# NikNazarov/TorchPIV

Hardware: AMD Instinct MI355X
Metric: image-pairs/sec at 4 MP, wind=64 ov=32 2-pass CWS; % HBM roofline (higher is better)
Workload: dtype u32 exact sums + f64 / f32

## Files before the change

### torchpiv_amd/csrc/xcorr_tile.hpp

```cpp
#pragma once
#include <hip/hip_runtime.h>
#include <stdint.h>

#include "fft_inreg.hpp"
#include "piv_kernels.h"

namespace tpiv {

template <int WS, bool PLANAR_ = false>
struct TileGeo {
    static constexpr int WPW = 64 / WS;
    static constexpr int TS = WS > 32 ? 32 : WS;
    static constexpr int PITCH = TS + 1;
    static constexpr int NT = 64 / TS;
    static constexpr int TILE = TS * PITCH;
    static constexpr bool PLANAR = PLANAR_;
    static constexpr int HROWS = WS / 2 + 1;
    static constexpr int HTILE = HROWS * PITCH;
    static constexpr int LDS_FLOATS = NT * TILE * (PLANAR ? 1 : 2);
    static constexpr int MAP_PITCH = WS + 1;
    static constexpr int NDW = WS / 4;
};

template <int CTRL>
__device__ __forceinline__ int dpp_i(int v) {
    return __builtin_amdgcn_update_dpp(0, v, CTRL, 0xF, 0xF, true);
}
template <int CTRL>
__device__ __forceinline__ float dpp_f(float v) {
    return __int_as_float(dpp_i<CTRL>(__float_as_int(v)));
}
constexpr int DPP_XOR1 = 0xB1;
constexpr int DPP_XOR2 = 0x4E;
constexpr int DPP_HALF_MIRROR = 0x141;
constexpr int DPP_ROW_MIRROR = 0x140;

template <int HALF>
__device__ __forceinline__ void partner2(int a, int& pa) {
    if constexpr (HALF == 1) pa = dpp_i<DPP_XOR1>(a);
    else if constexpr (HALF == 2) pa = dpp_i<DPP_XOR2>(a);
    else if constexpr (HALF == 4) pa = dpp_i<DPP_HALF_MIRROR>(a);
    else if constexpr (HALF == 8) pa = dpp_i<DPP_ROW_MIRROR>(a);
}

template <int WS, typename T, typename OP>
__device__ __forceinline__ T grp_reduce(T v, OP op) {
    static_assert(sizeof(T) == 4 || sizeof(T) == 8, "one or two dwords");
    constexpr int NW = sizeof(T) / 4;
    union U {
        T t;
        int w[NW];
    };
    static_for<0, 4>([&](auto sc) TPIV_LAMBDA_INLINE {
        constexpr int half = 1 << decltype(sc)::value;
        if constexpr (half < WS) {
            U a, b;
            a.t = v;
#pragma unroll
            for (int q = 0; q < NW; ++q) partner2<half>(a.w[q], b.w[q]);
            v = op(v, b.t);
        }
    });
    if constexpr (WS >= 32) {
        U a, x, y;
        a.t = v;
#pragma unroll
        for (int q = 0; q < NW; ++q) {
            auto r = __builtin_amdgcn_permlane16_swap((unsigned)a.w[q], (unsigned)a.w[q], false, false);
            x.w[q] = (int)r[0];
            y.w[q] = (int)r[1];
        }
        v = op(x.t, y.t);
    }
    if constexpr (WS >= 64) {
        U a, x, y;
        a.t = v;
#pragma unroll
        for (int q = 0; q < NW; ++q) {
            auto r = __builtin_amdgcn_permlane32_swap((unsigned)a.w[q], (unsigned)a.w[q], false, false);
            x.w[q] = (int)r[0];
            y.w[q] = (int)r[1];
        }
        v = op(x.t, y.t);
    }
    return v;
}

template <int WS>
__device__ __forceinline__ float grp_sum(float v) {
    return grp_reduce<WS>(v, [](float a, float b) TPIV_LAMBDA_INLINE { return a + b; });
}

template <int WS>
__device__ __forceinline__ float grp_min(float v) {
    return grp_reduce<WS>(v, [](float a, float b) TPIV_LAMBDA_INLINE { return fminf(a, b); });
}

__device__ __forceinline__ float fetch_clamped_t(const uint8_t* __restrict__ f, long long q, int HW) {
    q = q < 0 ? 0 : (q > (long long)(HW - 1) ? (long long)(HW - 1) : q);
    return (float)f[q];
}

__device__ __forceinline__ int f2i_sat_t(float v) {
    v = fminf(fmaxf(v, -1073741824.f), 1073741824.f);
    return (int)v;
}

template <int K, int N>
__device__ __forceinline__ float byte_f(const uint32_t (&d)[N]) {
    return (float)((d[K >> 2] >> (8 * (K & 3))) & 0xffu);
}

template <int N>
__device__ __forceinline__ void load_dwords(const uint8_t* __restrict__ p, uint32_t (&d)[N]) {
    __builtin_memcpy(&d[0], p, 4 * N);
}

__device__ __forceinline__ float bilerp_ref(float f11, float f21, float f12, float f22, float wx_up,
                                            float wx_dn, float wy_up, float wy_dn, bool degenerate) {
#pragma clang fp contract(off)
    float r = (f11 * wx_up) * wy_up;
    r = r + (f21 * wx_dn) * wy_up;
    r = r + (f12 * wx_up) * wy_dn;
    r = r + (f22 * wx_dn) * wy_dn;
    return degenerate ? f11 : r;
}

__device__ __forceinline__ float bilerp_ref_m(float f11, float f21, float f12, float f22, float wx_up,
                                              float wx_dn, float wy_up, float wy_dn, unsigned degenerate_mask) {
#pragma clang fp contract(off)
    float r = (f11 * wx_up) * wy_up;
    r = r + (f21 * wx_dn) * wy_up;
    r = r + (f12 * wx_up) * wy_dn;
    r = r + (f22 * wx_dn) * wy_dn;
    const unsigned bits = (degenerate_mask & __float_as_uint(f11)) | (~degenerate_mask & __float_as_uint(r));
    return __uint_as_float(bits);
}

#ifdef TPIV_STAMPS
#define TPIV_STAMP_DECL unsigned long long st_acc[16] = {}; unsigned long long st_prev = 0; unsigned st_iter = 0; \
    unsigned long long st_t0 = __builtin_amdgcn_s_memtime(), st_r0 = __builtin_amdgcn_s_memrealtime();
#define TPIV_STAMP_START                                                                  \
    do {                                                                                  \
        __builtin_amdgcn_sched_barrier(0);                                                \
        asm volatile("s_memtime %0\n\ts_waitcnt lgkmcnt(0)" : "=s"(st_prev)::"memory");    \
        __builtin_amdgcn_sched_barrier(0);                                                \
    } while (0)
#define TPIV_STAMP(i)                                                                     \
    do {                                                                                  \
        unsigned long long st_t;                                                          \
        __builtin_amdgcn_sched_barrier(0);                                                \
        asm volatile("s_memtime %0\n\ts_waitcnt lgkmcnt(0)" : "=s"(st_t)::"memory");       \
        __builtin_amdgcn_sched_barrier(0);                                                \
        st_acc[i] += st_t - st_prev;                                                      \
        st_prev = st_t;                                                                   \
    } while (0)
#define TPIV_STAMP_FLUSH(pp)                                                              \
    do {                                                                                  \
        if ((pp).stamps != nullptr && threadIdx.x == 0) {                                 \
            for (int q_ = 0; q_ < 16; ++q_) atomicAdd(&(pp).stamps[q_], st_acc[q_]);      \
            atomicAdd(&(pp).stamps[16], (unsigned long long)st_iter);                     \
            atomicAdd(&(pp).stamps[17], __builtin_amdgcn_s_memtime() - st_t0);            \
            atomicAdd(&(pp).stamps[18], __builtin_amdgcn_s_memrealtime() - st_r0);        \
        }                                                                                 \
    } while (0)
#else
#define TPIV_STAMP_DECL
#define TPIV_STAMP_START
#define TPIV_STAMP(i)
#define TPIV_STAMP_FLUSH(pp)
#endif

__device__ __forceinline__ int fast_div(int n, unsigned magic, int shift) {
    return (int)(((unsigned long long)(unsigned)n * magic) >> shift);
}
inline void fast_div_setup(unsigned d, unsigned& magic, int& shift) {
    int s_ = 0;
    while ((1ull << s_) < d) ++s_;
    shift = 31 + s_;
    magic = (unsigned)(((1ull << shift) + d - 1) / d);
}

__device__ __forceinline__ int fresh_lane() {
    int l = (int)__builtin_amdgcn_mbcnt_hi(~0u, __builtin_amdgcn_mbcnt_lo(~0u, 0u));
    asm volatile("" : "+v"(l));
    return l;
}

__device__ __forceinline__ void wave_sync() {
    __builtin_amdgcn_fence(__ATOMIC_ACQ_REL, "wavefront");
    __builtin_amdgcn_wave_barrier();
}

template <int WS, bool PLANAR, bool NOSWAP = false>
__device__ __forceinline__ void transpose_tile(cf (&a)[WS], float* lds, int lane) {
    using G = TileGeo<WS, PLANAR>;
    constexpr int P = G::PITCH;
    static_assert(!NOSWAP || WS == 64, "the swap-free form is a 64x64 one");
    cf* tile = reinterpret_cast<cf*>(lds);
    if constexpr (PLANAR && WS > 32) {
        if constexpr (!NOSWAP) {
            static_for<0, 32>([&](auto kc) TPIV_LAMBDA_INLINE {
                constexpr int k = decltype(kc)::value;
                constexpr int lo = FFT_POS<k, WS>, hi = FFT_POS<k + 32, WS>;
                auto rx = __builtin_amdgcn_permlane32_swap(__float_as_uint(a[lo].x), __float_as_uint(a[hi].x),
                                                           false, false);
                auto ry = __builtin_amdgcn_permlane32_swap(__float_as_uint(a[lo].y), __float_as_uint(a[hi].y),
                                                           false, false);
                a[lo].x = __uint_as_float(rx[0]);
                a[hi].x = __uint_as_float(rx[1]);
                a[lo].y = __uint_as_float(ry[0]);
                a[hi].y = __uint_as_float(ry[1]);
            });
        }
        float* t = lds + (lane >> 5) * G::TILE;
        const float* t2 = NOSWAP ? lds + ((lane >> 5) ^ 1) * G::TILE : t;
        const int i = lane & 31;
        auto plane = [&](auto comp) TPIV_LAMBDA_INLINE {
            constexpr bool Y = decltype(comp)::value;
            float lowhalf[32];
            wave_sync();
            static_for<0, 32>([&](auto kc) TPIV_LAMBDA_INLINE {
                constexpr int k = decltype(kc)::value;
                constexpr int src = FFT_POS<k, WS>;
                t[i * P + k] = Y ? a[src].y : a[src].x;
            });
            wave_sync();
#pragma unroll
            for (int r = 0; r < 32; ++r) lowhalf[r] = t[r * P + i];
            wave_sync();
            static_for<0, 32>([&](auto kc) TPIV_LAMBDA_INLINE {
                constexpr int k = decltype(kc)::value;
                constexpr int src = FFT_POS<k + 32, WS>;
                t[i * P + k] = Y ? a[src].y : a[src].x;
            });
            wave_sync();
#pragma unroll
            for (int r = 0; r < 32; ++r) {
                if constexpr (Y) {
                    a[32 + r].y = t2[r * P + i];
                    a[r].y = lowhalf[r];
                } else {
                    a[32 + r].x = t2[r * P + i];
                    a[r].x = lowhalf[r];
                }
            }
        };
        plane(std::false_type{});
        plane(std::true_type{});
    } else if constexpr (PLANAR) {
        float* t = lds + (lane / WS) * G::TILE;
        const int i = lane % WS;
        wave_sync();
        static_for<0, WS>([&](auto kc) TPIV_LAMBDA_INLINE {
            constexpr int k = decltype(kc)::value;
            t[i * P + k] = a[FFT_POS<k, WS>].x;
        });
        wave_sync();
#pragma unroll
        for (int r = 0; r < WS; ++r) a[r].x = t[r * P + i];
        wave_sync();
        static_for<0, WS>([&](auto kc) TPIV_LAMBDA_INLINE {
            constexpr int k = decltype(kc)::value;
            t[i * P + k] = a[FFT_POS<k, WS>].y;
        });
        wave_sync();
#pragma unroll
        for (int r = 0; r < WS; ++r) a[r].y = t[r * P + i];
    } else if constexpr (WS <= 32) {
        cf* t = tile + (lane / WS) * G::TILE;
        const int i = lane % WS;
        wave_sync();
        static_for<0, WS>([&](auto kc) TPIV_LAMBDA_INLINE {
            constexpr int k = decltype(kc)::value;
            t[i * P + k] = a[FFT_POS<k, WS>];
        });
        wave_sync();
#pragma unroll
        for (int r = 0; r < WS; ++r) a[r] = t[r * P + i];
    } else {
        static_assert(NOSWAP, "the complex 64x64 tile (the CWS kernel at two wavefronts per SIMD) is swap-free");
        cf* t = tile + (lane >> 5) * G::TILE;
        const int i = lane & 31;
        cf lowhalf[32];
        wave_sync();
        static_for<0, 32>([&](auto kc) TPIV_LAMBDA_INLINE {
            constexpr int k = decltype(kc)::value;
            t[i * P + k] = a[FFT_POS<k, WS>];
        });
        wave_sync();
#pragma unroll
        for (int r = 0; r < 32; ++r) lowhalf[r] = t[r * P + i];
        wave_sync();
        static_for<0, 32>([&](auto kc) TPIV_LAMBDA_INLINE {
            constexpr int k = decltype(kc)::value;
            t[i * P + k] = a[FFT_POS<k + 32, WS>];
        });
        wave_sync();
        const cf* t2 = tile + ((lane >> 5) ^ 1) * G::TILE;
#pragma unroll
        for (int r = 0; r < 32; ++r) a[32 + r] = t2[r * P + i];
#pragma unroll
        for (int r = 0; r < 32; ++r) a[r] = lowhalf[r];
    }
}

template <int WS, bool PLANAR>
__device__ __forceinline__ void transpose_half(const cf (&a)[WS], cf (&g)[WS / 2 + 1], float* lds, int lane) {
    static_assert(WS <= 32 || WS == 64, "one tile per window");
    using G = TileGeo<WS, PLANAR>;
    constexpr int P = G::PITCH, M = WS / 2;
    const int i = lane % WS;
    if constexpr (WS == 64) {
        static_assert(!PLANAR, "planar 64x64 tiles run the paired half inverse");
        constexpr int Q = M + 1;
        static_assert(WS * Q * 2 <= G::LDS_FLOATS, "half-spectrum plane fits the tile");
        cf b[WS];
        static_for<0, WS>([&](auto kc) TPIV_LAMBDA_INLINE {
            constexpr int k = decltype(kc)::value;
            b[k] = a[FFT_POS<k, WS>];
            asm volatile("" : "+v"(b[k].x), "+v"(b[k].y));
        });
        wave_sync();
        cf* t = reinterpret_cast<cf*>(lds);
        if (i <= M) {
            static_for<0, WS>([&](auto kc) TPIV_LAMBDA_INLINE {
                constexpr int k = decltype(kc)::value;
                t[k * Q + i] = b[k];
            });
        }
        wave_sync();
#pragma unroll
        for (int r = 0; r <= M; ++r) g[r] = t[i * Q + r];
    } else if constexpr (PLANAR) {
        float* t = lds + (lane / WS) * G::HTILE;
        wave_sync();
        if (i <= M) {
            static_for<0, WS>([&](auto kc) TPIV_LAMBDA_INLINE {
                constexpr int k = decltype(kc)::value;
                t[i * P + k] = a[FFT_POS<k, WS>].x;
            });
        }
        wave_sync();
#pragma unroll
        for (int r = 0; r <= M; ++r) g[r].x = t[r * P + i];
        wave_sync();
        if (i <= M) {
            static_for<0, WS>([&](auto kc) TPIV_LAMBDA_INLINE {
                constexpr int k = decltype(kc)::value;
                t[i * P + k] = a[FFT_POS<k, WS>].y;
            });
        }
        wave_sync();
#pragma unroll
        for (int r = 0; r <= M; ++r) g[r].y = t[r * P + i];
    } else {
        cf* t = reinterpret_cast<cf*>(lds) + (lane / WS) * G::HTILE;
        wave_sync();
        if (i <= M) {
            static_for<0, WS>([&](auto kc) TPIV_LAMBDA_INLINE {
                constexpr int k = decltype(kc)::value;
                t[i * P + k] = a[FFT_POS<k, WS>];
            });
        }
        wave_sync();
#pragma unroll
        for (int r = 0; r <= M; ++r) g[r] = t[r * P + i];
    }
}

template <int WS, bool PLANAR>
__device__ __forceinline__ void transpose_half_pairs(const cf (&h)[WS / 2], cf (&g)[WS / 2 + 1], float* lds, int lane) {
    static_assert(PLANAR && (WS == 32 || WS == 64), "planar tiles of 32 and 64");
    using G = TileGeo<WS, PLANAR>;
    constexpr int M = WS / 2, Q = M + 1;
    static_assert(64 * Q <= G::LDS_FLOATS, "the half-spectrum plane fits the tile");
    const int r = lane % WS;
    float* t = lds + (lane / WS) * (WS * Q);
    const bool odd = r > M;
    constexpr bool ZERO_ODD = WS == 32;
    const bool up = odd || (r == 0 && ZERO_ODD) || (r == M && !ZERO_ODD);
    float* wp = t + (odd ? WS - r : r) + (up ? Q : 0);
    const float sy = odd ? -1.0f : 1.0f;
    cf b[M];
    static_for<0, M>([&](auto mc) TPIV_LAMBDA_INLINE {
        constexpr int m = decltype(mc)::value;
        b[m] = h[FFT_POS<m, M>];
        asm volatile("" : "+v"(b[m].x), "+v"(b[m].y));
    });
    const int y = lane % WS;
    const float* rd = t + y * Q;
    const float* r0 = t + ((y & ~1) + (ZERO_ODD ? 1 : 0)) * Q;
    const float* rm = t + ((y & ~1) + (ZERO_ODD ? 0 : 1)) * Q + M;
    wave_sync();
    static_for<0, M>([&](auto mc) TPIV_LAMBDA_INLINE {
        constexpr int m = decltype(mc)::value;
        wp[2 * Q * m] = b[m].x;
    });
    wave_sync();
    g[0].x = r0[0];
#pragma unroll
    for (int k = 1; k < M; ++k) g[k].x = rd[k];
    g[M].x = rm[0];
    wave_sync();
    static_for<0, M>([&](auto mc) TPIV_LAMBDA_INLINE {
        constexpr int m = decltype(mc)::value;
        wp[2 * Q * m] = b[m].y * sy;
    });
    wave_sync();
    g[0].y = r0[0];
#pragma unroll
    for (int k = 1; k < M; ++k) g[k].y = rd[k];
    g[M].y = rm[0];
    if (y & 1) {
        g[0].x = g[0].y;
        g[M].x = g[M].y;
    }
}

struct ItemGeom {
    int pair, win, y0, x0;
    int active;
    size_t fidx;
};

template <int WS, int MODE>
struct RawRows;
template <int WS>
struct RawRows<WS, MODE_PASS1> {
    uint32_t a[WS / 4], b[WS / 4];
};
template <int WS>
struct RawRows<WS, MODE_DWS> {
    uint32_t a[WS / 4], b[WS / 4];
    long long qa, qb;
    int reg;
    int cls;
    int fix;
};
template <int WS>
struct CoopGeo {
    static constexpr int NROW = WS + 1;
    static constexpr int RPG = (WS + 1 + 15) / 16;
    static constexpr int LOADED = 16 * RPG;
    static constexpr int T = NROW * RPG;
    static constexpr int NCH = (T + WS - 1) / WS;
    static constexpr int PITCH4 = RPG | 1;
    static constexpr int PATCH4 = NROW * PITCH4;
    static constexpr int BLOCK4 = (2 * PATCH4 + 15) / 16 * 16;
    static constexpr int FLOATS = (64 / WS) * BLOCK4 * 4;
    static constexpr int LDS_FLOATS = FLOATS + (64 / WS) * (WS + 1) * 4;
    static_assert(RPG <= PITCH4, "patch row pitch");
    __device__ static __forceinline__ void chunk(int ci, int& j, int& part) {
        if constexpr (RPG == 2) {
            j = ci >> 1;
            part = ci & 1;
        } else if constexpr (RPG == 3) {
            j = (ci * 171) >> 9;
            part = ci - 3 * j;
        } else {
            static_assert(RPG == 5, "chunks per row");
            j = (ci * 205) >> 10;
            part = ci - 5 * j;
        }
    }
};
template <int WS>
struct CoopOff {
    int o[CoopGeo<WS>::NCH];
    __device__ __forceinline__ void init(int r, int W) {
#pragma unroll
        for (int k = 0; k < CoopGeo<WS>::NCH; ++k) {
            int j, part;
            CoopGeo<WS>::chunk(r + WS * k, j, part);
            o[k] = r + WS * k < CoopGeo<WS>::T ? j * W + 16 * part : 0;
        }
    }
};
template <int WS>
struct RawRows<WS, MODE_CWS> {
    uint32_t ca[CoopGeo<WS>::NCH][4], cb[CoopGeo<WS>::NCH][4];
    int reg;
    int cls;
    int fix;
};

struct CwsRow {
    float wya_up, wya_dn, wyb_up, wyb_dn;
    int dya, uya, dyb, uyb;
    int ydeg_a, ydeg_b;
};
__device__ __forceinline__ CwsRow cws_row(int gy, float vy) {
    CwsRow c;
    const float gyf = (float)gy;
    const float nya = gyf - vy, nyb = gyf + vy;
    const float uya_f = ceilf(nya), dya_f = floorf(nya);
    const float uyb_f = ceilf(nyb), dyb_f = floorf(nyb);
    c.uya = f2i_sat_t(uya_f);
    c.dya = f2i_sat_t(dya_f);
    c.uyb = f2i_sat_t(uyb_f);
    c.dyb = f2i_sat_t(dyb_f);
    c.wya_up = uya_f - nya;
    c.wya_dn = nya - dya_f;
// ... 571 lines not shown
        m = row_of_lane(rl) * WS + (cols ? (int)__builtin_ctzll(cols) : 0);
    }
    const int wv = p.val_win;
    int s[EXACT_MAX_SECOND] = {-1, -1, -1};
    {
        const unsigned long long ex = exclusion_row_mask<WS>(m, ys, wv);
        const int exl = (int)(unsigned)ex, exh = (int)(unsigned)(ex >> 32);
        int smax = -1;
        static_for<0, WS>([&](auto kc) TPIV_LAMBDA_INLINE {
            constexpr int xsft = decltype(kc)::value;
            constexpr int xo = (xsft + WS / 2) % WS;
            const int kill = __builtin_amdgcn_sbfe(xsft < 32 ? exl : exh, xsft & 31, 1);
            const int cnd = __float_as_int(__fsub_rn(row[xo], cmin)) | kill;
            smax = cnd > smax ? cnd : smax;
        });
        const int sall = grp_reduce<WS>(smax, [](int a, int b) TPIV_LAMBDA_INLINE { return a > b ? a : b; });
        const float thr = __int_as_float(sall) - band;
        unsigned long long rows = sall >= 0 ? wballot(smax >= 0 && __int_as_float(smax) >= thr) : 0ull;
        open = open || __popcll(rows) > EXACT_MAX_SECOND;
        int ns = 0;
        for (int it = 0; it < EXACT_MAX_SECOND; ++it) {
            if (!any_left(rows)) break;
            const bool on = mine_left(rows);
            const int rl = on ? (int)__builtin_ctzll(rows) : 0;
            rows &= rows - 1;
            const int yr = row_of_lane(rl);
            const unsigned long long exr = exclusion_row_mask<WS>(m, yr, wv);
            unsigned long long cols = wballot(__fsub_rn(park(rl), cmin) >= thr) & ~exr;
            cols = on ? cols : 0ull;
            for (int k = 0; k < WS; ++k) {
                if (!any_left(cols)) break;
                const bool has = mine_left(cols);
                const int q = yr * WS + (has ? (int)__builtin_ctzll(cols) : 0);
                cols &= cols - 1;
                s[0] = (has && ns == 0) ? q : s[0];
                s[1] = (has && ns == 1) ? q : s[1];
                s[2] = (has && ns == 2) ? q : s[2];
                ns += has ? 1 : 0;
            }
        }
        open = open || ns > EXACT_MAX_SECOND;
    }
    int n[EXACT_MAX_MIN] = {-1, -1, -1, -1};
    {
        const float thr = cmin + band;
        unsigned long long rows = wballot(rmin <= thr);
        bool over = __popcll(rows) > EXACT_MAX_MIN;
        int nn = 0;
        for (int it = 0; it < EXACT_MAX_MIN; ++it) {
            if (!any_left(rows)) break;
            const bool on = mine_left(rows);
            const int rl = on ? (int)__builtin_ctzll(rows) : 0;
            rows &= rows - 1;
            const int yr = row_of_lane(rl);
            unsigned long long cols = wballot(park(rl) <= thr);
            cols = on ? cols : 0ull;
            over = over || nn + __popcll(cols) > EXACT_MAX_MIN;
            for (int k = 0; k < EXACT_MAX_MIN; ++k) {
                if (!any_left(cols)) break;
                const bool has = mine_left(cols) && cols != 0ull && nn < EXACT_MAX_MIN;
                const int q = yr * WS + (cols ? (int)__builtin_ctzll(cols) : 0);
                cols &= cols - 1;
                n[0] = (has && nn == 0) ? q : n[0];
                n[1] = (has && nn == 1) ? q : n[1];
                n[2] = (has && nn == 2) ? q : n[2];
                n[3] = (has && nn == 3) ? q : n[3];
                nn += has ? 1 : 0;
            }
        }
        n[3] = over ? -2 : n[3];
    }
    if (r == 0 && active) {
        const int m_out = dead ? -2 : (open ? -1 : m);
        auto pack = [](int lo_, int hi_) TPIV_LAMBDA_INLINE { return ((unsigned)lo_ & 0xffffu) | ((unsigned)hi_ << 16); };
        uint4 rec;
        rec.x = pack(m_out, s[0]);
        rec.y = pack(s[1], s[2]);
        rec.z = pack(n[0], n[1]);
        rec.w = pack(n[2], n[3]);
        p.cand[fidx] = rec;
    }
}

template <int WS, int MODE, int OCC, bool FAST, bool CAND, int ROLE = 0>
__device__ __forceinline__ void xcorr_tile_body(const PassParams& p) {
    constexpr bool PLANAR = OCC > 2;
    using G = TileGeo<WS, PLANAR>;
    static_assert(WS == 8 || WS == 16 || WS == 32 || WS == 64, "tile sizes of this kernel");
    constexpr int RBH = 64 * (WS + 1) <= G::LDS_FLOATS ? 1 : 2;
    static_assert(MODE == MODE_PASS1 || 64 * (WS / RBH + 1) <= G::LDS_FLOATS,
                  "slow-path row buffer (shifted passes) must fit the tile LDS");
    constexpr int LDSF = (MODE == MODE_CWS && CoopGeo<WS>::LDS_FLOATS > G::LDS_FLOATS)
                             ? CoopGeo<WS>::LDS_FLOATS : G::LDS_FLOATS;
    __shared__ __attribute__((aligned(16))) float tile[LDSF];

    using TW = std::conditional_t<WS == 16, TwRegs<WS>, TwLiteral>;
    TW tw;
    if constexpr (!std::is_same<TW, TwLiteral>::value) tw.init();
    constexpr bool TWF_COL = FFT_TWIDDLE_FIRST && !(WS == 64 && MODE == MODE_PASS1);

    const int N = p.n_rows * p.n_cols;
    const int groups = (N + G::WPW - 1) / G::WPW;
    const bool listed = ROLE == 0 && MODE != MODE_PASS1 && p.list_mode != 0;
    const int items = listed ? __builtin_amdgcn_readfirstlane((int)*p.slow_count) : p.batch * groups;
    const int st = p.ws - p.ov;
    auto real_item = [&](int pos) TPIV_LAMBDA_INLINE { return listed ? __builtin_amdgcn_readfirstlane(p.slow_list[pos]) : pos; };

    constexpr int QCH = WS <= 16 ? 4 : 1;
    const int xcd = blockIdx.x & 7;
    const int chunk = (int)(((long long)items + 7) / 8);
    const int lo = __builtin_amdgcn_readfirstlane(xcd * chunk < items ? xcd * chunk : items);
    const int hi = __builtin_amdgcn_readfirstlane(items - lo > chunk ? lo + chunk : items);
    unsigned* const ctr = p.work_ctr + xcd * 16;
    int q_base = 0;
    int q_left = 0;
    auto q_issue = [&]() TPIV_LAMBDA_INLINE -> unsigned {
        unsigned v = 0;
        if (QCH == 1 || q_left == 0) {
            if (fresh_lane() == 0) v = atomicAdd(ctr, (unsigned)QCH);
        }
        return v;
    };
    auto q_take = [&](unsigned q_raw) TPIV_LAMBDA_INLINE -> int {
        if (QCH == 1 || q_left == 0) {
            const unsigned v = (unsigned)__builtin_amdgcn_readfirstlane((int)q_raw);
            q_base = v < (unsigned)(hi - lo) ? lo + (int)v : hi;
            q_left = QCH;
        }
        const int it = q_base + (QCH - q_left);
        --q_left;
        return it;
    };

    auto geom_of = [&](int pos, int w) TPIV_LAMBDA_INLINE {
        ItemGeom g;
        const int item = real_item(pos);
        g.pair = fast_div(item, p.groups_magic, p.groups_shift);
        const int gi = item - g.pair * groups;
        const int win_raw = gi * G::WPW + w;
        g.active = win_raw < N ? 1 : 0;
        g.win = g.active ? win_raw : N - 1;
        const int wrow = fast_div(g.win, p.ncols_magic, p.ncols_shift);
        g.y0 = wrow * st;
        g.x0 = (g.win - wrow * p.n_cols) * st;
        g.fidx = (size_t)g.pair * N + g.win;
        return g;
    };
    auto shift_of = [&](const ItemGeom& g, float& vx, float& vy) TPIV_LAMBDA_INLINE {
        if constexpr (MODE == MODE_PASS1) {
            vx = 0.f;
            vy = 0.f;
        } else {
            if constexpr (MODE == MODE_CWS) {
                pred_half_shift_cws_f32(p, g.fidx, vx, vy);
            } else {
                double sx, sy;
                pred_half_shift<MODE>(p, g.fidx, sx, sy);
                vx = (float)sx;
                vy = (float)sy;
            }
        }
    };

    int item = q_take(q_issue());
    if (item >= hi) return;
    int nitem = q_take(q_issue());
    constexpr bool RECOMPUTE = WS >= 32;
    float vx, vy;
    RawRows<WS, MODE> raw;
    ItemGeom gcur;
    CoopOff<WS> coff;
    if constexpr (MODE == MODE_CWS) coff.init(fresh_lane() % WS, p.W);
    {
        const int l0 = fresh_lane();
        gcur = geom_of(item, l0 / WS);
        shift_of(gcur, vx, vy);
        issue_rows<WS, MODE, FAST>(p, gcur, l0 % WS, vx, vy, raw, coff);
    }

    TPIV_STAMP_DECL
    TPIV_STAMP_START;
    for (int nnitem; item < hi; item = nitem, nitem = nnitem) {
        const unsigned q_raw = q_issue();
#ifdef TPIV_STAMPS
        ++st_iter;
#endif
        const int lane = fresh_lane();
        const int w = lane / WS;
        const int r = lane % WS;
        const ItemGeom g = RECOMPUTE ? geom_of(item, w) : gcur;
        const bool active = g.active != 0;
        const size_t fidx = g.fidx;
        const int nit = nitem < hi ? nitem : item;
        const ItemGeom gnext = geom_of(nit, w);
        float nvx, nvy;
        shift_of(gnext, nvx, nvy);

        if constexpr (ROLE == 1) {
            if (!raw.reg) {
                if (lane == 0) p.slow_list[atomicAdd(p.slow_count, 1u)] = item;
                nnitem = q_take(q_raw);
                issue_rows<WS, MODE, FAST>(p, gnext, r, nvx, nvy, raw, coff);
                vx = nvx;
                vy = nvy;
                if constexpr (!RECOMPUTE) gcur = gnext;
                continue;
            }
        }
        cf x[WS];
        float sa, sb;
        constexpr int NBS = WS >= 32 ? G::WPW : 1;
        int band_s[NBS];
        TPIV_STAMP(0);
        RowSquares sq;
        convert_rows<WS, MODE, RBH, FAST, CAND, ROLE == 1 ? 1 : 0>(p, g, r, lane, vx, vy, raw, x, sa, sb, tile, &sq);
        TPIV_STAMP(1);
        if constexpr (WS >= 64) nnitem = q_take(q_raw);
        if constexpr (WS <= 32) issue_rows<WS, MODE, FAST>(p, gnext, r, nvx, nvy, raw, coff);

        if (p.dbg_win != nullptr && active) {
            int rr = r;
            asm volatile("" : "+v"(rr));
            float* d = p.dbg_win + fidx * 2 * WS * WS + rr * WS;
#pragma unroll
            for (int k = 0; k < WS; ++k) {
                d[k] = x[k].x;
                d[WS * WS + k] = x[k].y;
            }
        }

        bool dead = false;
        float end_scale = 1.0f;
        constexpr bool FASTN = FAST && MODE != MODE_PASS1;
        constexpr bool NOSWAP = WS == 64 && !(MODE == MODE_DWS && FAST);
        auto up_sign = []() TPIV_LAMBDA_INLINE { return fresh_lane() >= 32 ? 0x80000000u : 0u; };
        auto sflip = [](float v, unsigned sg) TPIV_LAMBDA_INLINE { return __uint_as_float(__float_as_uint(v) ^ sg); };
        if constexpr (!FASTN) {
            sa = grp_sum<WS>(sa);
            sb = grp_sum<WS>(sb);
            const float ma = sa * (1.0f / (WS * WS)), mb = sb * (1.0f / (WS * WS));
            float ka = 1.f, kb = 1.f;
            if constexpr (MODE == MODE_PASS1) {
                dead = (sa == 0.f) || (sb == 0.f);
                ka = dead ? 0.f : 1.0f / ma;
                kb = dead ? 0.f : 1.0f / mb;
            }
            if constexpr (CAND) {
                auto uadd = [](unsigned a_, unsigned b_) TPIV_LAMBDA_INLINE { return a_ + b_; };
                const unsigned saa = grp_reduce<WS>(sq.aa, uadd), sbb = grp_reduce<WS>(sq.bb, uadd);
                constexpr double NN = (double)(WS * WS);
                const double da = (double)sa, db = (double)sb;
                const float ea = (float)__fma_rn(-da, da, NN * (double)saa), eb = (float)__fma_rn(-db, db, NN * (double)sbb);
                const float e_plus = (0.5f / (float)(WS * WS)) * (ea * (ka * ka) + eb * (kb * kb));
                const float bnd = dead ? 0.f : p.exact_band * e_plus;
                if constexpr (WS >= 32) {
                    static_for<0, G::WPW>([&](auto wc) TPIV_LAMBDA_INLINE {
                        band_s[decltype(wc)::value] = __builtin_amdgcn_readlane(__float_as_int(bnd), decltype(wc)::value * WS);
                    });
                } else {
                    band_s[0] = __float_as_int(bnd);
                }
            }
            constexpr float PRE = 0.5f / (float)WS;
            const float oa = -ma * ka, ob = -mb * kb;
            const float kas = ka * PRE, kbs = kb * PRE, oas = oa * PRE, obs = ob * PRE;
            const unsigned sg = NOSWAP ? up_sign() : 0u;
            const float kao = sflip(kas, sg), kbo = sflip(kbs, sg), oao = sflip(oas, sg), obo = sflip(obs, sg);
#pragma unroll
            for (int k = 0; k < WS; ++k) {
                x[k].x = (k & 1) ? fmaf(x[k].x, kao, oao) : fmaf(x[k].x, kas, oas);
                x[k].y = (k & 1) ? fmaf(x[k].y, kbo, obo) : fmaf(x[k].y, kbs, obs);
            }
        } else if constexpr (NOSWAP) {
            const unsigned sg = up_sign();
#pragma unroll
            for (int k = 1; k < WS; k += 2) {
                x[k].x = sflip(x[k].x, sg);
                x[k].y = sflip(x[k].y, sg);
            }
        }

        TPIV_STAMP(2);
        fft_inreg<WS, 1>(x, tw);
        if constexpr (FASTN) {
            constexpr int P0 = FFT_POS<0, WS>;
            if constexpr (NOSWAP) {
                constexpr int PH = FFT_POS<WS / 2, WS>;
                const bool up = up_sign() != 0u;
                const float ta = grp_sum<WS>(up ? x[PH].x : x[P0].x);
                const float tb = grp_sum<WS>(up ? x[PH].y : x[P0].y);
                x[P0].x -= up ? 0.0f : ta * (1.0f / WS);
                x[P0].y -= up ? 0.0f : tb * (1.0f / WS);
                x[PH].x -= up ? ta * (1.0f / WS) : 0.0f;
                x[PH].y -= up ? tb * (1.0f / WS) : 0.0f;
            } else {
                const float ta = grp_sum<WS>(x[P0].x);
                const float tb = grp_sum<WS>(x[P0].y);
                x[P0].x -= ta * (1.0f / WS);
                x[P0].y -= tb * (1.0f / WS);
            }
            end_scale = 0.25f / (float)(WS * WS);
        }
        TPIV_STAMP(3);
        transpose_tile<WS, PLANAR, NOSWAP>(x, tile, fresh_lane());
        TPIV_STAMP(4);
        fft_inreg<WS, 1, TW, TWF_COL>(x, tw);
        TPIV_STAMP(5);

        constexpr bool HALF_INV = PLANAR && (WS == 32 || WS == 64);
        float crow[WS];
        if constexpr (HALF_INV) {
            constexpr int M = WS / 2;
            cf h[M];
            {
                const int lane_c = fresh_lane();
                const int r_c = lane_c % WS;
                const int partner = (lane_c - r_c) + ((WS - r_c) % WS);
                auto cross = [&](cf zk, cf zm, float two) TPIV_LAMBDA_INLINE {
                    const float a_ = zk.x, b_ = zk.y, c_ = zm.x, d_ = zm.y;
                    cf pr;
                    pr.x = (a_ * d_ + b_ * c_) * two;
                    pr.y = (c_ * c_ - a_ * a_) + (d_ * d_ - b_ * b_);
                    return pr;
                };
                const float two_odd = (NOSWAP && (lane_c & 31) != 0) ? -2.0f : 2.0f;
                cf pc[M + 1];
                static_for<0, M + 1>([&](auto kc) TPIV_LAMBDA_INLINE {
                    constexpr int ky = decltype(kc)::value;
                    constexpr int nky = (WS - ky) % WS;
                    const cf z2 = x[FFT_POS<nky, WS>];
                    cf m1;
                    m1.x = __shfl(z2.x, partner, 64);
                    m1.y = __shfl(z2.y, partner, 64);
                    pc[ky] = cross(x[FFT_POS<ky, WS>], m1, (ky & 1) ? two_odd : 2.0f);
                });
                TPIV_STAMP(6);
                const bool odd = r_c > M;
                const float fs = (r_c == 0 || r_c == M) ? 1.0f : 0.0f;
                static_for<0, M>([&](auto kc) TPIV_LAMBDA_INLINE {
                    constexpr int k = decltype(kc)::value;
                    cf pr;
                    pr.x = __shfl(pc[M - k].x, partner, 64);
                    pr.y = __shfl(pc[M - k].y, partner, 64);
                    const cf s{pc[k].x + pr.x, pc[k].y - pr.y};
                    const cf tt = twmul<k, WS, -1>(cf{pc[k].x - pr.x, pc[k].y + pr.y});
                    h[k].x = odd ? tt.x : __builtin_fmaf(-fs, tt.y, s.x);
                    h[k].y = odd ? tt.y : __builtin_fmaf(fs, tt.x, s.y);
                });
            }
            fft_inreg<M, -1>(h, tw);
            TPIV_STAMP(7);
            cf hs[M + 1], z[M];
            transpose_half_pairs<WS, PLANAR>(h, hs, tile, fresh_lane());
            TPIV_STAMP(8);
            c2r_inreg<WS>(hs, z);
            static_for<0, WS>([&](auto xc) TPIV_LAMBDA_INLINE {
                constexpr int x_ = decltype(xc)::value;
                crow[x_] = (x_ & 1) ? z[FFT_POS<x_ / 2, M>].y : z[FFT_POS<x_ / 2, M>].x;
            });
        } else {
            {
                const int lane_c = fresh_lane();
                const int r_c = lane_c % WS;
                const int partner = (lane_c - r_c) + ((WS - r_c) % WS);
                auto cross = [&](cf zk, cf zm, float two) TPIV_LAMBDA_INLINE {
                    const float a_ = zk.x, b_ = zk.y, c_ = zm.x, d_ = zm.y;
                    cf pr;
                    pr.x = (a_ * d_ + b_ * c_) * two;
                    pr.y = (c_ * c_ - a_ * a_) + (d_ * d_ - b_ * b_);
                    return pr;
                };
                const float two_odd = (NOSWAP && (lane_c & 31) != 0) ? -2.0f : 2.0f;
                static_for<0, WS / 2 + 1>([&](auto kc) TPIV_LAMBDA_INLINE {
                    constexpr int ky = decltype(kc)::value;
                    constexpr int nky = (WS - ky) % WS;
                    constexpr int p1 = FFT_POS<ky, WS>, p2 = FFT_POS<nky, WS>;
                    const float two = (ky & 1) ? two_odd : 2.0f;
                    const cf z1 = x[p1];
                    if constexpr (ky == nky) {
                        cf m1;
                        m1.x = __shfl(z1.x, partner, 64);
                        m1.y = __shfl(z1.y, partner, 64);
                        x[p1] = cross(z1, m1, two);
                    } else {
                        const cf z2 = x[p2];
                        cf m1, m2;
                        m1.x = __shfl(z2.x, partner, 64);
                        m1.y = __shfl(z2.y, partner, 64);
                        m2.x = __shfl(z1.x, partner, 64);
                        m2.y = __shfl(z1.y, partner, 64);
                        x[p1] = cross(z1, m1, two);
                        x[p2] = cross(z2, m2, two);
                    }
                });
            }

            TPIV_STAMP(6);
            cf t[WS];
            static_for<0, WS>([&](auto kc) TPIV_LAMBDA_INLINE {
                constexpr int ky = decltype(kc)::value;
                t[ky] = x[FFT_POS<ky, WS>];
            });
            fft_inreg<WS, -1>(t, tw);
            TPIV_STAMP(7);
            cf hs[WS / 2 + 1], z[WS / 2];
            transpose_half<WS, PLANAR>(t, hs, tile, fresh_lane());
            TPIV_STAMP(8);
            c2r_inreg<WS>(hs, z);
            static_for<0, WS>([&](auto xc) TPIV_LAMBDA_INLINE {
                constexpr int x_ = decltype(xc)::value;
                crow[x_] = (x_ & 1) ? z[FFT_POS<x_ / 2, WS / 2>].y : z[FFT_POS<x_ / 2, WS / 2>].x;
            });
        }
        wave_sync();
        TPIV_STAMP(9);

        auto band_of = [&](int w_) TPIV_LAMBDA_INLINE {
            int b_ = band_s[0];
            static_for<1, NBS>([&](auto wc) TPIV_LAMBDA_INLINE { b_ = w_ == decltype(wc)::value ? band_s[decltype(wc)::value] : b_; });
            return __int_as_float(b_);
        };
        if constexpr (WS > 32) {
            const int lane_p = fresh_lane();
            issue_rows<WS, MODE, FAST>(p, geom_of(nit, lane_p / WS), lane_p % WS, nvx, nvy, raw, coff);
        }
        vx = nvx;
        vy = nvy;
        if constexpr (!RECOMPUTE) gcur = gnext;

        TPIV_STAMP(10);
        if constexpr (RECOMPUTE) {
            const int lane_e = fresh_lane();
            const int w_e = lane_e / WS, r_e = lane_e % WS;
            const int item_e = real_item(item);
            const int pair_e = fast_div(item_e, p.groups_magic, p.groups_shift);
            const int win_raw_e = (item_e - pair_e * groups) * G::WPW + w_e;
            const bool active_e = win_raw_e < N;
            const int win_e = active_e ? win_raw_e : N - 1;
            const size_t fidx_e = (size_t)pair_e * N + win_e;
            if constexpr (CAND) peak_candidates<WS>(p, crow, tile, w_e, r_e, active_e, dead, fidx_e, band_of(w_e));
            else peak_analysis<WS, PLANAR, FASTN>(p, crow, tile, w_e, r_e, active_e, dead, fidx_e, end_scale);
        } else {
            if constexpr (CAND) peak_candidates<WS>(p, crow, tile, w, r, active, dead, fidx, band_of(w));
            else peak_analysis<WS, PLANAR, FASTN>(p, crow, tile, w, r, active, dead, fidx, end_scale);
        }
        wave_sync();
        if constexpr (WS < 64) nnitem = q_take(q_raw);
        TPIV_STAMP(13);
    }
    TPIV_STAMP_FLUSH(p);
}

template <int WS, int MODE, int OCC, bool FAST>
__global__ __launch_bounds__(64, OCC) void xcorr_tile_kernel(PassParams p) {
    xcorr_tile_body<WS, MODE, OCC, FAST, false>(p);
}
template <int WS, int MODE>
__global__ __launch_bounds__(64, 3) void xcorr_tile_fastpath_kernel(PassParams p) {
    xcorr_tile_body<WS, MODE, 3, true, false, 1>(p);
}
template <int WS>
__global__ __launch_bounds__(64, tile_occ_c(WS, MODE_PASS1)) void xcorr_tile_cand_kernel(PassParams p) {
    xcorr_tile_body<WS, MODE_PASS1, tile_occ_c(WS, MODE_PASS1), true, true>(p);
}

template <int WS, bool PLANAR>
__global__ __launch_bounds__(64, 2) void peak_debug_kernel(PassParams p, const float* maps, int n_maps) {
    using G = TileGeo<WS, PLANAR>;
    __shared__ float tile[G::LDS_FLOATS];
    const int lane = threadIdx.x;
    const int w = lane / WS, r = lane % WS;
    const int win_raw = blockIdx.x * G::WPW + w;
    const bool active = win_raw < n_maps;
    const int win = active ? win_raw : n_maps - 1;
    float crow[WS];
    const int ys = (r + WS / 2) % WS;
#pragma unroll
    for (int xo = 0; xo < WS; ++xo) crow[xo] = maps[((size_t)win * WS + ys) * WS + (xo + WS / 2) % WS];
    peak_analysis<WS, PLANAR>(p, crow, tile, w, r, active, false, (size_t)win);
}

template <int WS>
hipError_t launch_peak_debug(const PassParams& p, const float* maps, int n_maps, int planar, hipStream_t stream) {
    using G = TileGeo<WS, false>;
    const int blocks = (n_maps + G::WPW - 1) / G::WPW;
    if (planar)
        hipLaunchKernelGGL((peak_debug_kernel<WS, true>), dim3(blocks), dim3(64), 0, stream, p, maps, n_maps);
    else
        hipLaunchKernelGGL((peak_debug_kernel<WS, false>), dim3(blocks), dim3(64), 0, stream, p, maps, n_maps);
    return hipGetLastError();
}

template <int WS>
static unsigned tile_grid(PassParams& p, int n_cu) {
    using G = TileGeo<WS>;
    const int N = p.n_rows * p.n_cols;
    const long long groups = (N + G::WPW - 1) / G::WPW;
    const long long items = (long long)p.batch * groups;
    if (items <= 0 || items >= (1ll << 31) - 64) return 0;
    fast_div_setup((unsigned)groups, p.groups_magic, p.groups_shift);
    fast_div_setup((unsigned)p.n_cols, p.ncols_magic, p.ncols_shift);
    const long long cap = (long long)n_cu * 64;
    const long long blocks = items < cap ? items : cap;
    return (unsigned)((blocks + 7) / 8 * 8);
}

template <int WS, int MODE>
static hipError_t launch_tile(const PassParams& p_in, int n_cu, hipStream_t stream) {
    PassParams p = p_in;
    const unsigned blocks = tile_grid<WS>(p, n_cu);
    if (blocks == 0) return hipErrorInvalidValue;
    constexpr int OCC = tile_occ_c(WS, MODE);
    if constexpr (MODE != MODE_PASS1) {
        if (p.precision != 0) {
            hipLaunchKernelGGL((xcorr_tile_kernel<WS, MODE, OCC, false>), dim3(blocks), dim3(64), 0, stream, p);
            return hipGetLastError();
        }
    }
    if constexpr (tile_split64(WS, MODE)) {
        if (p.slow_list != nullptr && p.slow_count != nullptr) {
            hipLaunchKernelGGL((xcorr_tile_fastpath_kernel<WS, MODE>), dim3(blocks), dim3(64), 0, stream, p);
            hipError_t e_ = hipGetLastError();
            if (e_ != hipSuccess) return e_;
            e_ = hipMemsetAsync(p.work_ctr, 0, TILE_CTR_BYTES, stream);
            if (e_ != hipSuccess) return e_;
            PassParams q = p;
            q.list_mode = 1;
            long long blocks2 = (long long)n_cu * 8;
            if (blocks2 > blocks) blocks2 = blocks;
            blocks2 = (blocks2 + 7) / 8 * 8;
            hipLaunchKernelGGL((xcorr_tile_kernel<WS, MODE, OCC, true>), dim3((unsigned)blocks2), dim3(64), 0, stream, q);
            return hipGetLastError();
        }
    }
    hipLaunchKernelGGL((xcorr_tile_kernel<WS, MODE, OCC, true>), dim3(blocks), dim3(64), 0, stream, p);
    return hipGetLastError();
}

template <int WS>
hipError_t launch_xcorr_tile_cand_ws(const PassParams& p_in, int n_cu, hipStream_t stream) {
    PassParams p = p_in;
    const unsigned blocks = tile_grid<WS>(p, n_cu);
    if (blocks == 0 || p.cand == nullptr) return hipErrorInvalidValue;
    hipLaunchKernelGGL((xcorr_tile_cand_kernel<WS>), dim3(blocks), dim3(64), 0, stream, p);
    return hipGetLastError();
}

template <int WS>
hipError_t launch_xcorr_tile_ws(const PassParams& p, int mode, int n_cu, hipStream_t stream) {
    switch (mode) {
        case MODE_PASS1: return launch_tile<WS, MODE_PASS1>(p, n_cu, stream);
        case MODE_DWS: return launch_tile<WS, MODE_DWS>(p, n_cu, stream);
        case MODE_CWS: return launch_tile<WS, MODE_CWS>(p, n_cu, stream);
        default: return hipErrorInvalidValue;
    }
}

}
```

Before: 18950.

## Transpose planar tiles through lane-contiguous LDS rows with ds_write_addtid

```diff
diff --git a/torchpiv_amd/csrc/xcorr_tile.hpp b/torchpiv_amd/csrc/xcorr_tile.hpp
--- a/torchpiv_amd/csrc/xcorr_tile.hpp
+++ b/torchpiv_amd/csrc/xcorr_tile.hpp
@@ -17,7 +17,9 @@
     static constexpr bool PLANAR = PLANAR_;
     static constexpr int HROWS = WS / 2 + 1;
     static constexpr int HTILE = HROWS * PITCH;
-    static constexpr int LDS_FLOATS = NT * TILE * (PLANAR ? 1 : 2);
+    static constexpr int ROW_PITCH = 68;
+    static constexpr int ROW_FLOATS = (PLANAR && WS >= 32) ? 32 * ROW_PITCH : 0;
+    static constexpr int LDS_FLOATS = NT * TILE * (PLANAR ? 1 : 2) > ROW_FLOATS ? NT * TILE * (PLANAR ? 1 : 2) : ROW_FLOATS;
     static constexpr int MAP_PITCH = WS + 1;
     static constexpr int NDW = WS / 4;
 };
@@ -192,13 +194,93 @@
     __builtin_amdgcn_wave_barrier();
 }
 
-template <int WS, bool PLANAR, bool NOSWAP = false>
+template <int WS, int E0, int R0, bool Y>
+__device__ __forceinline__ void store_rows16(const cf (&a)[WS], float* lds) {
+    constexpr int P = TileGeo<WS, true>::ROW_PITCH;
+    static_assert(P == 68, "the offsets below are 272 * row");
+    const unsigned m0 = __builtin_amdgcn_readfirstlane((unsigned)(uintptr_t)lds) + 4u * P * R0;
+    unsigned keep;
+#define TPIV_ROW(q) "v"(Y ? a[FFT_POS<E0 + R0 + q, WS>].y : a[FFT_POS<E0 + R0 + q, WS>].x)
+    asm volatile(
+        "s_mov_b32 %0, m0\n\t"
+        "s_mov_b32 m0, %1\n\t"
+        "s_nop 0\n\t"
+        "ds_write_addtid_b32 %2 offset:0\n\t"
+        "ds_write_addtid_b32 %3 offset:272\n\t"
+        "ds_write_addtid_b32 %4 offset:544\n\t"
+        "ds_write_addtid_b32 %5 offset:816\n\t"
+        "ds_write_addtid_b32 %6 offset:1088\n\t"
+        "ds_write_addtid_b32 %7 offset:1360\n\t"
+        "ds_write_addtid_b32 %8 offset:1632\n\t"
+        "ds_write_addtid_b32 %9 offset:1904\n\t"
+        "ds_write_addtid_b32 %10 offset:2176\n\t"
+        "ds_write_addtid_b32 %11 offset:2448\n\t"
+        "ds_write_addtid_b32 %12 offset:2720\n\t"
+        "ds_write_addtid_b32 %13 offset:2992\n\t"
+        "ds_write_addtid_b32 %14 offset:3264\n\t"
+        "ds_write_addtid_b32 %15 offset:3536\n\t"
+        "ds_write_addtid_b32 %16 offset:3808\n\t"
+        "ds_write_addtid_b32 %17 offset:4080\n\t"
+        "s_mov_b32 m0, %0"
+        : "=&s"(keep)
+        : "s"(m0), TPIV_ROW(0), TPIV_ROW(1), TPIV_ROW(2), TPIV_ROW(3), TPIV_ROW(4), TPIV_ROW(5), TPIV_ROW(6), TPIV_ROW(7),
+          TPIV_ROW(8), TPIV_ROW(9), TPIV_ROW(10), TPIV_ROW(11), TPIV_ROW(12), TPIV_ROW(13), TPIV_ROW(14), TPIV_ROW(15)
+        : "memory");
+#undef TPIV_ROW
+}
+__device__ __forceinline__ void read_row32(const float* src, float (&v)[32]) {
+    const float4* s4 = reinterpret_cast<const float4*>(src);
+#pragma unroll
+    for (int n = 0; n < 8; ++n) {
+        const float4 q = s4[n];
+        v[4 * n] = q.x;
+        v[4 * n + 1] = q.y;
+        v[4 * n + 2] = q.z;
+        v[4 * n + 3] = q.w;
+    }
+}
+
+template <int WS, bool PLANAR, bool NOSWAP = false, bool ROWS = false>
 __device__ __forceinline__ void transpose_tile(cf (&a)[WS], float* lds, int lane) {
     using G = TileGeo<WS, PLANAR>;
     constexpr int P = G::PITCH;
     static_assert(!NOSWAP || WS == 64, "the swap-free form is a 64x64 one");
+    static_assert(!ROWS || (PLANAR && (WS == 32 || (WS == 64 && NOSWAP))), "lane-contiguous tiles: planar 32x32 and swap-free 64x64");
     cf* tile = reinterpret_cast<cf*>(lds);
-    if constexpr (PLANAR && WS > 32) {
+    if constexpr (ROWS) {
+        static_assert(32 * G::ROW_PITCH <= G::LDS_FLOATS, "the lane-contiguous tile fits");
+        const float* rd1 = lds + (lane & 31) * G::ROW_PITCH + 32 * (lane >> 5);
+        auto plane = [&](auto comp) TPIV_LAMBDA_INLINE {
+            constexpr bool Y = decltype(comp)::value;
+            float got[32];
+            wave_sync();
+            store_rows16<WS, 0, 0, Y>(a, lds);
+            store_rows16<WS, 0, 16, Y>(a, lds);
+            wave_sync();
+            read_row32(rd1, got);
+            if constexpr (WS == 64) {
+                const float* rd2 = lds + (lane & 31) * G::ROW_PITCH + 32 * ((lane >> 5) ^ 1);
+                float high[32];
+                wave_sync();
+                store_rows16<WS, 32, 0, Y>(a, lds);
+                store_rows16<WS, 32, 16, Y>(a, lds);
+                wave_sync();
+                read_row32(rd2, high);
+#pragma unroll
+                for (int r = 0; r < 32; ++r) {
+                    if constexpr (Y) a[32 + r].y = high[r];
+                    else a[32 + r].x = high[r];
+                }
+            }
+#pragma unroll
+            for (int r = 0; r < 32; ++r) {
+                if constexpr (Y) a[r].y = got[r];
+                else a[r].x = got[r];
+            }
+        };
+        plane(std::false_type{});
+        plane(std::true_type{});
+    } else if constexpr (PLANAR && WS > 32) {
         if constexpr (!NOSWAP) {
             static_for<0, 32>([&](auto kc) TPIV_LAMBDA_INLINE {
                 constexpr int k = decltype(kc)::value;
@@ -1376,7 +1458,8 @@
             end_scale = 0.25f / (float)(WS * WS);
         }
         TPIV_STAMP(3);
-        transpose_tile<WS, PLANAR, NOSWAP>(x, tile, fresh_lane());
+        constexpr bool ROWS = PLANAR && (WS == 32 || NOSWAP);
+        transpose_tile<WS, PLANAR, NOSWAP, ROWS>(x, tile, fresh_lane());
         TPIV_STAMP(4);
         fft_inreg<WS, 1, TW, TWF_COL>(x, tw);
         TPIV_STAMP(5);
```

After: 19380 (median of 6 runs). 2.3% higher.
